# AIM-Harvard/pyradiomics

Measured on NVIDIA H100. Metric: voxels/s full-texture voxel-based, higher is better.
Workload: dtype f64

## Files before the change

### pyradiomics_b200/csrc/glrlm_fast.cuh

```cuda
#pragma once
#include "glcm_fast.cuh"

namespace rb {

struct GlrlmFastTables {
  uint32_t VA[GF_NA], VA2[GF_NA];
  uint8_t delta[GF_NA];
  double log2t[32];
  double clog2[32];
  double inv2[256];
};

inline void glrlm_fast_build_tables(GlrlmFastTables& T) {
  int ang[13][3], k = 0;
  for (int z = 1; z >= -1; z--) for (int y = 1; y >= -1; y--) for (int x = 1; x >= -1; x--)
    if (k < 13) { ang[k][0] = z; ang[k][1] = y; ang[k][2] = x; k++; }
  for (int a = 0; a < 13; a++) {
    T.VA[a] = T.VA2[a] = 0;
    T.delta[a] = (uint8_t)(ang[a][0] * 9 + ang[a][1] * 3 + ang[a][2]);
    for (int z = 0; z < 3; z++) for (int y = 0; y < 3; y++) for (int x = 0; x < 3; x++) {
      const int v = z * 9 + y * 3 + x;
      auto pos = [&](int m) {
        const int z2 = z + m * ang[a][0], y2 = y + m * ang[a][1], x2 = x + m * ang[a][2];
        return (z2 < 0 || z2 > 2 || y2 < 0 || y2 > 2 || x2 < 0 || x2 > 2) ? 31 : z2 * 9 + y2 * 3 + x2;
      };
      const int nx = pos(1), nx2 = pos(2);
      if (nx != 31) T.VA[a] |= 1u << v;
      if (nx2 != 31) T.VA2[a] |= 1u << v;
    }
  }
  T.log2t[0] = 0;
  T.clog2[0] = 0;
  for (int c = 1; c < 32; c++) { T.log2t[c] = log2((double)c); T.clog2[c] = c * log2((double)c); }
  T.inv2[0] = 0;
  for (int g = 1; g < 256; g++) T.inv2[g] = 1.0 / ((double)g * g);
}

RB_HD void glrlm_fast_voxel(const int* wl, const GlrlmFastTables& T, double* out) {
  uint32_t e[27];
  RB_EQMASKS_27(wl, e);
  uint32_t M = 0;
  uint32_t cls[13];
  int clg[13];
  int nl = 0;
  int S_n = 0, S_g = 0, S_g2 = 0;
  double S_ig = 0;
#pragma unroll
  for (int v = 0; v < 27; v++) {
    if (wl[v]) M |= 1u << v;
    if (e[v] && (e[v] & ((1u << v) - 1)) == 0) {
      if (e[v] == (1u << v)) { S_n++; S_g += wl[v]; S_g2 += wl[v] * wl[v]; S_ig += T.inv2[wl[v]]; }
      else { cls[nl] = e[v]; clg[nl] = wl[v]; nl++; }
    }
  }
  const int Np = RB_POPC(M);
  double sum[GLRLM_NF];
#pragma unroll
  for (int k = 0; k < GLRLM_NF; k++) sum[k] = 0;
  int nang = 0;
  for (int a = 0; a < GF_NA; a++) {
    const int d = T.delta[a];
    const uint32_t VA = T.VA[a];
    if (!(((M & VA) & (M >> d)) | ((M & T.VA2[a]) & (M >> (2 * d))))) continue;
    uint32_t NS = 0;
    for (int k = 0; k < nl; k++) NS |= cls[k] & (cls[k] >> d);
    NS &= VA;
    const uint32_t ENDS = M & ~NS, PS = NS << d, PS2 = PS & (PS << d);
    const uint32_t L1 = ENDS & ~PS, L2 = ENDS & PS & ~PS2, L3 = ENDS & PS2;
    const int n1 = RB_POPC(L1), n2 = RB_POPC(L2), n3 = RB_POPC(L3);
    int B1 = S_g2, B2 = 0, B3 = 0, C = S_g, sg = S_n;
    double A1 = S_ig, A2 = 0, A3 = 0, lg = 0;
    for (int k = 0; k < nl; k++) {
      const uint32_t E = cls[k];
      const int c1 = RB_POPC(E & L1), c2 = RB_POPC(E & L2), c3 = RB_POPC(E & L3), ce = c1 + c2 + c3;
      const int g = clg[k], g2 = g * g;
      const double ig = T.inv2[g];
      sg += ce * ce; C += ce * g;
      B1 += c1 * g2; B2 += c2 * g2; B3 += c3 * g2;
      A1 += c1 * ig; A2 += c2 * ig; A3 += c3 * ig;
      lg += T.clog2[c1] + T.clog2[c2] + T.clog2[c3];
    }
    const int Nr = n1 + n2 + n3;
    const double invNr = 1.0 / Nr, invNr2 = invNr * invNr;
    const int lre_n = n1 + 4 * n2 + 9 * n3, B = B1 + B2 + B3;
    sum[R_ShortRunEmphasis] += (n1 + n2 * 0.25 + n3 * (1.0 / 9.0)) * invNr;
    sum[R_LongRunEmphasis] += lre_n * invNr;
    sum[R_GrayLevelNonUniformity] += sg * invNr;
    sum[R_GrayLevelNonUniformityNormalized] += sg * invNr2;
    const int rl = n1 * n1 + n2 * n2 + n3 * n3;
    sum[R_RunLengthNonUniformity] += rl * invNr;
    sum[R_RunLengthNonUniformityNormalized] += rl * invNr2;
    sum[R_RunPercentage] += (double)Nr / Np;
    sum[R_GrayLevelVariance] += (double)(Nr * B - C * C) * invNr2;
    sum[R_RunVariance] += (double)(Nr * lre_n - Np * Np) * invNr2;
    sum[R_RunEntropy] += T.log2t[Nr] - lg * invNr;
    sum[R_LowGrayLevelRunEmphasis] += (A1 + A2 + A3) * invNr;
    sum[R_HighGrayLevelRunEmphasis] += B * invNr;
    sum[R_ShortRunLowGrayLevelEmphasis] += (A1 + A2 * 0.25 + A3 * (1.0 / 9.0)) * invNr;
    sum[R_ShortRunHighGrayLevelEmphasis] += (B1 + B2 * 0.25 + B3 * (1.0 / 9.0)) * invNr;
    sum[R_LongRunLowGrayLevelEmphasis] += (A1 + 4.0 * A2 + 9.0 * A3) * invNr;
    sum[R_LongRunHighGrayLevelEmphasis] += (double)(B1 + 4 * B2 + 9 * B3) * invNr;
    nang++;
  }
  const double inv = nang ? 1.0 / nang : NAN;
#pragma unroll
  for (int k = 0; k < GLRLM_NF; k++) out[k] = nang ? sum[k] * inv : NAN;
}

}
```

### pyradiomics_b200/csrc/small_fast.cuh

```cuda
#pragma once
#include "glcm_fast.cuh"

namespace rb {

struct SmallFastTables {
  double log2t[32];
  double inv2[256];
  double invsq[32];
  double rcp[64];
};

inline void small_fast_build_tables(SmallFastTables& T) {
  T.log2t[0] = 0; T.invsq[0] = 0; T.inv2[0] = 0; T.rcp[0] = 0;
  for (int c = 1; c < 32; c++) { T.log2t[c] = log2((double)c); T.invsq[c] = 1.0 / ((double)c * c); }
  for (int g = 1; g < 256; g++) T.inv2[g] = 1.0 / ((double)g * g);
  for (int c = 1; c < 64; c++) T.rcp[c] = 1.0 / (double)c;
}

RB_HD constexpr uint32_t nb26(int v) {
  uint32_t m = 0;
  const int z = v / 9, y = (v / 3) % 3, x = v % 3;
  for (int dz = -1; dz <= 1; dz++) for (int dy = -1; dy <= 1; dy++) for (int dx = -1; dx <= 1; dx++) {
    if (!dz && !dy && !dx) continue;
    const int z2 = z + dz, y2 = y + dy, x2 = x + dx;
    if (z2 < 0 || z2 > 2 || y2 < 0 || y2 > 2 || x2 < 0 || x2 > 2) continue;
    m |= 1u << (z2 * 9 + y2 * 3 + x2);
  }
  return m;
}
template <int V> struct NB26 { static constexpr uint32_t value = nb26(V); };

template <int V, int END> struct ForPos {
  template <typename F> static RB_HD void go(F& f) { f.template at<V>(); ForPos<V + 1, END>::go(f); }
};
template <int END> struct ForPos<END, END> { template <typename F> static RB_HD void go(F&) {} };

struct GldmPass1 {
  const int* wl; const uint32_t* cl; int* dep; uint32_t M;
  template <int V> RB_HD void at() { dep[V] = wl[V] ? (int)RB_POPC(cl[V] & NB26<V>::value) : -1 - V; }
};

RB_HD void gldm_fast_voxel(const int* wl, int alpha, const SmallFastTables& T, double* out) {
  uint32_t eq[27];
  RB_EQMASKS_27(wl, eq);
  uint32_t cl[27];
  if (alpha == 0) {
#pragma unroll
    for (int v = 0; v < 27; v++) cl[v] = eq[v];
  } else {
#pragma unroll
    for (int v = 0; v < 27; v++) cl[v] = 0;
#pragma unroll
    for (int p = 0; p < 27; p++)
#pragma unroll
      for (int q = p + 1; q < 27; q++) {
        const int d = wl[p] - wl[q];
        if (wl[p] && wl[q] && d <= alpha && -d <= alpha) { cl[p] |= 1u << q; cl[q] |= 1u << p; }
      }
  }
  int dep[27];
  GldmPass1 p1{wl, cl, dep, 0};
  ForPos<0, 27>::go(p1);
  uint32_t dq[27];
  RB_EQMASKS_27_KEY(dep, dq);
  int Nz = 0, Sj = 0, Sj2 = 0, B = 0, C = 0, X4 = 0, gl = 0, dn = 0;
  double Sinv = 0, A = 0, X1 = 0, X2 = 0, X3 = 0, lg = 0;
#pragma unroll
  for (int v = 0; v < 27; v++) {
    if (wl[v]) {
      const int g = wl[v], g2 = g * g, j = dep[v] + 1, j2 = j * j;
      const double ig = T.inv2[g], ij = T.invsq[j];
      Nz++; Sj += j; Sj2 += j2; B += g2; C += g; X4 += g2 * j2;
      Sinv += ij; A += ig; X1 += ig * ij; X2 += g2 * ij; X3 += j2 * ig;
      gl += RB_POPC(eq[v]); dn += RB_POPC(dq[v]);
      lg += T.log2t[RB_POPC(eq[v] & dq[v])];
    }
  }
  const double inv = 1.0 / Nz, inv2 = inv * inv;
  out[0] = T.log2t[Nz] - lg * inv;
  out[1] = dn * inv;
  out[2] = dn * inv2;
  out[3] = (double)(Nz * Sj2 - Sj * Sj) * inv2;
  out[4] = gl * inv;
  out[5] = (double)(Nz * B - C * C) * inv2;
  out[6] = B * inv;
  out[7] = Sj2 * inv;
  out[8] = X4 * inv;
  out[9] = X3 * inv;
  out[10] = A * inv;
  out[11] = Sinv * inv;
  out[12] = X2 * inv;
  out[13] = X1 * inv;
}

constexpr int NGTDM_L = 34034;

RB_HD constexpr int ngtdm_full_cnt(int v) {
  return (v % 3 == 1 ? 3 : 2) * ((v / 3) % 3 == 1 ? 3 : 2) * (v / 9 == 1 ? 3 : 2) - 1;
}

RB_HD double ngtdm_i2d(int d) {
#ifdef __CUDA_ARCH__
  return __hiloint2double(0x43300000, d) - 4503599627370496.0;
#else
  return (double)d;
#endif
}

RB_HD double ngtdm_complexity_pairs(const int* pk, const double* ns, int st, int nl, const SmallFastTables& T) {
  double c0 = 0, c1 = 0;
  for (int a = 0; a + 1 < nl; a++) {
    const int pa = pk[a * st], na = pa >> 8, ia = pa & 255;
    const double sa = ns[a * st];
    int b = a + 1;
    for (; b + 1 < nl; b += 2) {
      const int p0 = pk[b * st], p1 = pk[(b + 1) * st];
      const int x0 = ia - (p0 & 255), x1 = ia - (p1 & 255);
      c0 += ngtdm_i2d(x0 < 0 ? -x0 : x0) * ((sa + ns[b * st]) * T.rcp[na + (p0 >> 8)]);
      c1 += ngtdm_i2d(x1 < 0 ? -x1 : x1) * ((sa + ns[(b + 1) * st]) * T.rcp[na + (p1 >> 8)]);
    }
    if (b < nl) {
      const int p0 = pk[b * st], x0 = ia - (p0 & 255);
      c0 += ngtdm_i2d(x0 < 0 ? -x0 : x0) * ((sa + ns[b * st]) * T.rcp[na + (p0 >> 8)]);
    }
  }
  return c0 + c1;
}

struct NgtdmGeneralDiff {
  const int* wl; const uint32_t* eq; uint32_t M; const SmallFastTables* T; double* scr_ns; int st; double ssum;
  template <int V> RB_HD void at() {
    if (!wl[V]) return;
    constexpr uint32_t nb = NB26<V>::value;
    int sum = 0;
#pragma unroll
    for (int u = 0; u < 27; u++) if (nb >> u & 1u) sum += wl[u];
    const int cnt = RB_POPC(M & nb), x = cnt * wl[V] - sum;
    const double d = ngtdm_i2d(x < 0 ? -x : x) * T->rcp[cnt];
    ssum += d;
    const int r = RB_CTZ(eq[V]);
    const double prev = r == V ? 0.0 : scr_ns[r * st];
    scr_ns[r * st] = prev + d;
  }
};

template <bool FULL>
RB_HD void ngtdm_fast_body(const int* wl, const SmallFastTables& T, double* out, int* scr_pk, double* scr_ns, int st) {
  int B = 0, C = 0;
#pragma unroll
  for (int v = 0; v < 27; v++) { B += wl[v] * wl[v]; C += wl[v]; }
  uint32_t eq[27];
  RB_EQMASKS_27(wl, eq);
  int Nvp = 27, SE = 0;
  double ssum = 0;
  if (FULL) {
    int bx[27], by[27], bz[27];
#pragma unroll
    for (int r = 0; r < 27; r += 3) {
      bx[r] = wl[r] + wl[r + 1]; bx[r + 1] = bx[r] + wl[r + 2]; bx[r + 2] = wl[r + 1] + wl[r + 2];
    }
#pragma unroll
    for (int r = 0; r < 27; r += 9)
#pragma unroll
      for (int x = 0; x < 3; x++) {
        const int* b = bx + r + x;
        by[r + x] = b[0] + b[3]; by[r + 3 + x] = by[r + x] + b[6]; by[r + 6 + x] = b[3] + b[6];
      }
#pragma unroll
    for (int yx = 0; yx < 9; yx++) {
      bz[yx] = by[yx] + by[9 + yx]; bz[9 + yx] = bz[yx] + by[18 + yx]; bz[18 + yx] = by[9 + yx] + by[18 + yx];
    }
#pragma unroll
    for (int v = 0; v < 27; v++) {
      const int cnt = ngtdm_full_cnt(v);
      const int x = (cnt + 1) * wl[v] - bz[v];
      const int e = (x < 0 ? -x : x) * (NGTDM_L / cnt);
      SE += e;
      const int r = RB_CTZ(eq[v]);
      const int prev = r == v ? 0 : scr_pk[r * st];
      scr_pk[r * st] = prev + e;
    }
  } else {
    uint32_t M = 0;
#pragma unroll
    for (int v = 0; v < 27; v++) if (wl[v]) M |= 1u << v;
    Nvp = RB_POPC(M);
    NgtdmGeneralDiff p1{wl, eq, M, &T, scr_ns, st, 0.0};
    ForPos<0, 27>::go(p1);
    ssum = p1.ssum;
  }
  int nl = 0, SL = 0, SL2 = 0;
  double pw = 0;
  int X[27];
#pragma unroll
  for (int v = 0; v < 27; v++) {
    const bool rep = eq[v] && (eq[v] & ((1u << v) - 1)) == 0;
    const int n = RB_POPC(eq[v]), g = wl[v];
    const double ns = FULL ? ngtdm_i2d(n) * ngtdm_i2d(scr_pk[v * st]) : ngtdm_i2d(n) * scr_ns[v * st];
    scr_pk[nl * st] = n << 8 | g;
    scr_ns[nl * st] = ns;
    X[v] = rep ? g * n : 0;
    if (rep) { nl++; SL += g; SL2 += g * g; pw += ns; }
  }
  RB_NGTDM_SORT27(X);
  int bd = 0;
#pragma unroll
  for (int k = 0; k < 27; k++) bd += (2 * k - 53 + nl) * X[k];
  const double cpx = ngtdm_complexity_pairs(scr_pk, scr_ns, st, nl, T);
  const double u = FULL ? (double)NGTDM_L : 1.0, N = (double)Nvp;
  const double sdiff = FULL ? (double)SE : ssum;
  out[N_Coarseness] = pw != 0 ? N * u / pw : 1e6;
  const double div = (double)nl * (nl - 1);
  out[N_Contrast] = div != 0 ? 2.0 * (double)(Nvp * B - C * C) * sdiff / (N * N * N * u * div) : 0.0;
  out[N_Busyness] = bd != 0 ? pw / (2.0 * u * (double)bd) : 0.0;
  out[N_Complexity] = 2.0 * cpx / (N * u);
  out[N_Strength] = sdiff != 0 ? 2.0 * u * (double)(nl * B - 2 * C * SL + Nvp * SL2) / (N * sdiff) : 0.0;
}

RB_HD bool ngtdm_window_full(const int* wl) {
  bool full = true;
#pragma unroll
  for (int v = 0; v < 27; v++) full &= wl[v] != 0;
  return full;
}

RB_HD void ngtdm_fast_voxel(const int* wl, const SmallFastTables& T, double* out) {
  int pk[27] = {0};
  double ns[27] = {0};
  if (ngtdm_window_full(wl)) ngtdm_fast_body<true>(wl, T, out, pk, ns, 1);
  else ngtdm_fast_body<false>(wl, T, out, pk, ns, 1);
}

RB_HD uint32_t dilate26(uint32_t m) {
  constexpr uint32_t X0 = 0x1249249u, X2 = 0x4924924u;
  constexpr uint32_t Y0 = 0x01C0E07u, Y2 = 0x70381C0u;
  m |= ((m & ~X2) << 1) | ((m & ~X0) >> 1);
  m |= ((m & ~Y2) << 3) | ((m & ~Y0) >> 3);
  m |= (m << 9) | (m >> 9);
  return m & 0x7FFFFFFu;
}

struct GlszmAcc {
  int Nz, Sg, Sg2, Ss2, X4, gln;
  double A, Sinv, X1, X2, X3, lg;
  unsigned long long h0, h1, h2;
};

RB_HD void glszm_fast_voxel(const int* wl, const SmallFastTables& T, double* out) {
  uint32_t eq[27];
  RB_EQMASKS_27(wl, eq);
  uint32_t M = 0;
  uint32_t cls[13];
  int clg[13];
  int nl = 0, S_n = 0, S_g = 0, S_g2 = 0;
  double S_ig = 0;
#pragma unroll
  for (int v = 0; v < 27; v++) {
    if (wl[v]) M |= 1u << v;
    if (eq[v] && (eq[v] & ((1u << v) - 1)) == 0) {
      if (eq[v] == (1u << v)) { S_n++; S_g += wl[v]; S_g2 += wl[v] * wl[v]; S_ig += T.inv2[wl[v]]; }
      else { cls[nl] = eq[v]; clg[nl] = wl[v]; nl++; }
    }
  }
  GlszmAcc a;
  a.Nz = S_n; a.Sg = S_g; a.Sg2 = S_g2; a.Ss2 = S_n; a.X4 = S_g2; a.gln = S_n;
  a.A = S_ig; a.Sinv = (double)S_n; a.X1 = S_ig; a.X2 = (double)S_g2; a.X3 = S_ig; a.lg = 0;
  a.h0 = (unsigned long long)S_n; a.h1 = a.h2 = 0;
  for (int k = 0; k < nl; k++) {
    const int g = clg[k], g2 = g * g;
    uint32_t m = cls[k];
    const double ig = T.inv2[g];
    int zs[8];
    int zc = 0;
    while (m && zc < 8) {
      uint32_t comp = m & (0u - m);
      for (;;) {
        const uint32_t nx = dilate26(comp) & m;
        if (nx == comp) break;
        comp = nx;
      }
      m &= ~comp;
      const int sz = RB_POPC(comp), s2 = sz * sz;
      zs[zc++] = sz;
      const double is = T.invsq[sz];
      a.Nz++; a.Sg += g; a.Sg2 += g2; a.Ss2 += s2; a.X4 += g2 * s2;
      a.A += ig; a.Sinv += is; a.X1 += ig * is; a.X2 += g2 * is; a.X3 += s2 * ig;
      if (sz <= 12) a.h0 += 1ull << (5 * (sz - 1));
      else if (sz <= 24) a.h1 += 1ull << (5 * (sz - 13));
      else a.h2 += 1ull << (5 * (sz - 25));
    }
    a.gln += zc * zc;
    for (int k = 0; k < zc; k++) {
      int c = 0;
      for (int l = 0; l < zc; l++) c += zs[l] == zs[k];
      a.lg += T.log2t[c];
    }
  }
  int szn = 0;
#pragma unroll
  for (int k = 0; k < 12; k++) {
    const int c0 = (int)(a.h0 >> (5 * k)) & 31, c1 = (int)(a.h1 >> (5 * k)) & 31;
    szn += c0 * c0 + c1 * c1;
  }
#pragma unroll
  for (int k = 0; k < 3; k++) { const int c2 = (int)(a.h2 >> (5 * k)) & 31; szn += c2 * c2; }
  const int Np = RB_POPC(M), Nz = a.Nz;
  const double inv = 1.0 / Nz, inv2 = inv * inv;
  out[S_GLN] = a.gln * inv; out[S_GLNN] = a.gln * inv2;
  out[S_GLV] = (double)(Nz * a.Sg2 - a.Sg * a.Sg) * inv2;
  out[S_HGLE] = a.Sg2 * inv; out[S_LargeE] = a.Ss2 * inv; out[S_LargeHGLE] = a.X4 * inv; out[S_LargeLGLE] = a.X3 * inv;
  out[S_LGLE] = a.A * inv; out[S_SizeNU] = szn * inv; out[S_SizeNUN] = szn * inv2; out[S_SmallE] = a.Sinv * inv;
  out[S_SmallHGLE] = a.X2 * inv; out[S_SmallLGLE] = a.X1 * inv;
  out[S_Entropy] = T.log2t[Nz] - a.lg * inv;
  out[S_Percentage] = (double)Nz / Np;
  out[S_SizeVar] = (double)(Nz * a.Ss2 - Np * Np) * inv2;
}

}
```

### pyradiomics_b200/csrc/voxel_fast.cu

```cuda
#include <map>
#include <mutex>

#include "common.cuh"
#define RB_GLCM_BLOCK_SYNC 1
#include "glcm_fast.cuh"
#include "glcm_kernels.cuh"
#include "glrlm_fast.cuh"
#include "small_fast.cuh"
#include "host_common.hpp"

namespace rb {

bool glcm_fast_applicable(int cls, int level_bytes, const VoxParams& P) {
  return cls == C_GLCM && level_bytes == 1 && P.rz == 1 && P.ry == 1 && P.rx == 1 && P.na == 13 && P.symmetric &&
         !P.weighted && P.Ng <= 255;
}

struct GlcmQueue { GlcmTask* q = nullptr; double* res = nullptr; unsigned* count = nullptr; size_t cap = 0; };
static std::mutex g_queue_mu;
static std::map<std::pair<int, cudaStream_t>, GlcmQueue> g_queue_cache;
int glcm_release_queues() {
  int dev = 0;
  if (cudaGetDevice(&dev) != cudaSuccess) return RB_ERR_CUDA;
  cudaDeviceSynchronize();
  std::lock_guard<std::mutex> lk(g_queue_mu);
  for (auto it = g_queue_cache.begin(); it != g_queue_cache.end();) {
    if (it->first.first == dev) {
      cudaFree(it->second.q); cudaFree(it->second.res); cudaFree(it->second.count);
      it = g_queue_cache.erase(it);
    } else ++it;
  }
  return RB_OK;
}
static GlcmQueue* glcm_queue(cudaStream_t st, size_t need) {
  std::mutex& mu = g_queue_mu;
  auto& cache = g_queue_cache;
  int dev = 0;
  if (cudaGetDevice(&dev) != cudaSuccess) return nullptr;
  std::lock_guard<std::mutex> lk(mu);
  GlcmQueue& Q = cache[{dev, st}];
  if (!Q.count && cudaMalloc(&Q.count, sizeof(unsigned)) != cudaSuccess) return nullptr;
  if (Q.cap < need) {
    if (Q.q) { cudaStreamSynchronize(st); cudaFree(Q.q); cudaFree(Q.res); Q.q = nullptr; Q.res = nullptr; Q.cap = 0; }
    if (cudaMalloc(&Q.q, need * sizeof(GlcmTask)) != cudaSuccess) return nullptr;
    if (cudaMalloc(&Q.res, need * sizeof(double)) != cudaSuccess) { cudaFree(Q.q); Q.q = nullptr; return nullptr; }
    Q.cap = need;
  }
  return &Q;
}

int glcm_fast_launch(const void* lev, const uint8_t* centers, const VoxParams& P, double* out, long long fstride,
                     int z0, int z1, int out_z0, cudaStream_t st) {
  const GlcmFastTables* T = device_table<GlcmFastTables>([&](GlcmFastTables& h) { glcm_fast_build_tables(h, P.Ng); }, P.Ng);
  if (!T) return fail(RB_ERR_CUDA, "could not build the GLCM table block on the device");
  const long long plane = (long long)P.Y * P.X;
  if ((long long)(z1 - z0) * plane <= 0) return RB_OK;
  if (P.sy != P.X || P.sz != plane) return fail(RB_ERR_ARG, "GLCM fast path expects a contiguous level volume");
  const int sms = sm_count();
  const long long max_entries = 48ll << 20;
  int zchunk = (int)(max_entries / (plane * GF_NA));
  if (zchunk < 1) zchunk = 1;
  if (zchunk > z1 - z0) zchunk = z1 - z0;
  GlcmQueue* Q = glcm_queue(st, (size_t)zchunk * plane * GF_NA);
  if (!Q) return fail(RB_ERR_NOMEM, "could not allocate the GLCM eigen-task queue");
  constexpr int NT = 512;
  const int smem = glcm_phaseA_smem_bytes(NT);
  RB_CUDA(set_max_dynamic_smem(glcm_fast_kernel<1, NT>, smem));
  RB_CUDA(set_max_dynamic_smem(glcm_fast_solve_kernel<2>, GF_LZ_SMEM_BYTES));
  const uint8_t* l8 = (const uint8_t*)lev;
  for (int za = z0; za < z1; za += zchunk) {
    const int zb = za + zchunk < z1 ? za + zchunk : z1;
    RB_CUDA(cudaMemsetAsync(Q->count, 0, sizeof(unsigned), st));
    int grid = 0;
    RB_CUDA(resident_grid(glcm_fast_kernel<1, NT>, NT, smem, (long long)(zb - za) * plane, grid));
    glcm_fast_kernel<1, NT><<<grid, NT, smem, st>>>(l8, centers, P, T, out, fstride, za, zb, out_z0, Q->q, Q->count);
    RB_LAUNCH_CHECK();
    glcm_fast_solve_kernel<0><<<sms * 8, 128, 0, st>>>(l8, P, T, Q->q, Q->count, Q->res, 0);
    for (int g = 10; g <= 12; g += 2) glcm_fast_solve_kernel<1><<<sms * 8, 128, 0, st>>>(l8, P, T, Q->q, Q->count, Q->res, g);
    for (int g = 18; g >= 14; g -= 2)
      glcm_fast_solve_kernel<2><<<sms * 2, 128, GF_LZ_SMEM_BYTES, st>>>(l8, P, T, Q->q, Q->count, Q->res, g);
    RB_LAUNCH_CHECK();
    glcm_fast_finish_kernel<<<sms * 8, 256, 0, st>>>(P, Q->q, Q->count, Q->res, out + (long long)G_MCC * fstride, out_z0);
    RB_LAUNCH_CHECK();
  }
  return RB_OK;
}

__global__ void __launch_bounds__(128)
glrlm_fast_kernel(const uint8_t* __restrict__ lev, const uint8_t* __restrict__ centers,
                  const __grid_constant__ VoxParams P, const GlrlmFastTables* __restrict__ Tg,
                  double* __restrict__ out, long long fstride, int z0, int z1, int out_z0) {
  __shared__ GlrlmFastTables T;
  copy_tables_to_shared(T, Tg);
  __syncthreads();
  const long long plane = (long long)P.Y * P.X;
  const long long total = (long long)(z1 - z0) * plane;
  for (long long t = (long long)blockIdx.x * blockDim.x + threadIdx.x; t < total; t += (long long)gridDim.x * blockDim.x) {
    const ChunkVoxel v = chunk_voxel(P, plane, z0, out_z0, t);
    if (!chunk_center(lev, centers, plane, v)) {
#pragma unroll
      for (int k = 0; k < GLRLM_NF; k++) out[k * fstride + v.oi] = P.init_value;
      continue;
    }
    int wl[27];
    load_window27(lev, P, v.z, v.y, v.x, v.vi, true, wl, 1);
    double f[GLRLM_NF];
    glrlm_fast_voxel(wl, T, f);
#pragma unroll
    for (int k = 0; k < GLRLM_NF; k++) out[k * fstride + v.oi] = f[k];
  }
}

bool glrlm_fast_applicable(int cls, int level_bytes, const VoxParams& P) {
  return cls == C_GLRLM && level_bytes == 1 && P.rz == 1 && P.ry == 1 && P.rx == 1 && P.na == 13 && !P.weighted && P.Ng <= 255;
}

int glrlm_fast_launch(const void* lev, const uint8_t* centers, const VoxParams& P, double* out, long long fstride,
                      int z0, int z1, int out_z0, cudaStream_t st) {
  const GlrlmFastTables* T = device_table<GlrlmFastTables>(glrlm_fast_build_tables);
  if (!T) return fail(RB_ERR_CUDA, "could not build the GLRLM table block on the device");
  const long long total = (long long)(z1 - z0) * P.Y * P.X;
  if (total <= 0) return RB_OK;
  glrlm_fast_kernel<<<grid_for(total, 128, 32), 128, 0, st>>>((const uint8_t*)lev, centers, P, T, out, fstride, z0, z1, out_z0);
  RB_LAUNCH_CHECK();
  return RB_OK;
}

template <int CLS, int NT, bool SYNC>
__global__ void __launch_bounds__(NT)
small_fast_kernel(const uint8_t* __restrict__ lev, const uint8_t* __restrict__ centers,
                  const __grid_constant__ VoxParams P, const SmallFastTables* __restrict__ Tg,
                  double* __restrict__ out, long long fstride, int z0, int z1, int out_z0) {
  __shared__ SmallFastTables T;
  copy_tables_to_shared<NT>(T, Tg);
  __syncthreads();
  constexpr int NF = CLS == C_GLSZM ? GLSZM_NF : GLDM_NF;
  const long long plane = (long long)P.Y * P.X;
  const long long total = (long long)(z1 - z0) * plane;
  const long long ntiles = (total + NT - 1) / NT;
  for (long long tile = blockIdx.x; tile < ntiles; tile += gridDim.x) {
    if (SYNC) __syncthreads();
    const long long t = tile * NT + threadIdx.x;
    const bool live = t < total;
    if (!SYNC && !live) continue;
    const ChunkVoxel v = chunk_voxel(P, plane, z0, out_z0, t, live);
    const bool is_center = live && chunk_center(lev, centers, plane, v);
    if (!SYNC && !is_center) {
#pragma unroll
      for (int k = 0; k < NF; k++) out[k * fstride + v.oi] = P.init_value;
      continue;
    }
    int wl[27];
    load_window27(lev, P, v.z, v.y, v.x, v.vi, is_center, wl, 1);
    double f[16];
    if (CLS == C_GLSZM) glszm_fast_voxel(wl, T, f);
    else gldm_fast_voxel(wl, P.alpha, T, f);
    if (!live) continue;
#pragma unroll
    for (int k = 0; k < NF; k++) out[k * fstride + v.oi] = is_center ? f[k] : P.init_value;
  }
}

constexpr int NGTDM_NT = 128;
template <int NT>
__global__ void __launch_bounds__(NT, 4)
ngtdm_fast_kernel(const uint8_t* __restrict__ lev, const uint8_t* __restrict__ centers,
                  const __grid_constant__ VoxParams P, const SmallFastTables* __restrict__ Tg,
                  double* __restrict__ out, long long fstride, int z0, int z1, int out_z0) {
  __shared__ SmallFastTables T;
  __shared__ double ng_ns[27 * NT];
  __shared__ int ng_pk[27 * NT];
  __shared__ long long defer[2 * NT];
  __shared__ unsigned ndefer;
  copy_tables_to_shared<NT>(T, Tg);
  const int tid = threadIdx.x;
  if (tid == 0) ndefer = 0;
  __syncthreads();
  const long long plane = (long long)P.Y * P.X;
  full_window_tiles<NT>((long long)(z1 - z0) * plane, defer, ndefer,
    [&](long long t, bool live, auto defer_it) {
      if (!live) return;
      const ChunkVoxel v = chunk_voxel(P, plane, z0, out_z0, t);
      const bool is_center = chunk_center(lev, centers, plane, v);
      int wl[27];
      load_window27(lev, P, v.z, v.y, v.x, v.vi, is_center, wl, 1);
      if (is_center && ngtdm_window_full(wl)) {
        double f[NGTDM_NF];
        ngtdm_fast_body<true>(wl, T, f, ng_pk + tid, ng_ns + tid, NT);
#pragma unroll
        for (int k = 0; k < NGTDM_NF; k++) out[k * fstride + v.oi] = f[k];
      } else if (is_center) {
        defer_it();
      } else {
#pragma unroll
        for (int k = 0; k < NGTDM_NF; k++) out[k * fstride + v.oi] = P.init_value;
      }
    },
    [&](auto entry, bool live) {
      if (!live) return;
      const ChunkVoxel v = chunk_voxel(P, plane, z0, out_z0, entry());
      const bool is_center = chunk_center(lev, centers, plane, v);
      int wl[27];
      load_window27(lev, P, v.z, v.y, v.x, v.vi, is_center, wl, 1);
      double f[NGTDM_NF];
      ngtdm_fast_body<false>(wl, T, f, ng_pk + tid, ng_ns + tid, NT);
#pragma unroll
      for (int k = 0; k < NGTDM_NF; k++) out[k * fstride + v.oi] = f[k];
    });
}

bool small_fast_applicable(int cls, int level_bytes, const VoxParams& P) {
  return (cls == C_GLSZM || cls == C_GLDM || cls == C_NGTDM) && level_bytes == 1 && P.rz == 1 && P.ry == 1 && P.rx == 1 &&
         P.na == 26 && P.Ng <= 255;
}

int small_fast_launch(int cls, const void* lev, const uint8_t* centers, const VoxParams& P, double* out, long long fstride,
                      int z0, int z1, int out_z0, cudaStream_t st) {
  const SmallFastTables* T = device_table<SmallFastTables>(small_fast_build_tables);
  if (!T) return fail(RB_ERR_CUDA, "could not build the table block on the device");
  const long long total = (long long)(z1 - z0) * P.Y * P.X;
  if (total <= 0) return RB_OK;
  const uint8_t* l8 = (const uint8_t*)lev;
  if (cls == C_NGTDM) {
    int grid = 0;
    RB_CUDA(resident_grid(ngtdm_fast_kernel<NGTDM_NT>, NGTDM_NT, 0, total, grid));
    ngtdm_fast_kernel<NGTDM_NT><<<grid, NGTDM_NT, 0, st>>>(l8, centers, P, T, out, fstride, z0, z1, out_z0);
  } else if (cls == C_GLSZM) {
    small_fast_kernel<C_GLSZM, 128, false><<<grid_for(total, 128, 32), 128, 0, st>>>(l8, centers, P, T, out, fstride, z0, z1, out_z0);
  } else {
    small_fast_kernel<C_GLDM, 256, true><<<grid_for(total, 256, 16), 256, 0, st>>>(l8, centers, P, T, out, fstride, z0, z1, out_z0);
  }
  RB_LAUNCH_CHECK();
  return RB_OK;
}

}
```

Before: 263.9 million.

## Specialize GLRLM/GLSZM for full windows with deferred partial windows and shared scratch

Templates the GLRLM and GLSZM per-voxel bodies on a FULL flag so fully-populated 3x3x3 windows skip mask building and angle-skip tests. Both now run in the deferred-tile kernel used for NGTDM: partial-window voxels are queued and processed separately, which keeps warps convergent. Per-thread class masks move to strided shared memory to relieve registers. Reciprocal tables replace divisions, and GLSZM entropy uses an incremental nibble histogram instead of an O(n^2) recount. In exchange it adds shared-memory use and deferral synchronization, and the load_window27 return value is now treated as a fullness flag.

```diff
diff --git a/pyradiomics_b200/csrc/glrlm_fast.cuh b/pyradiomics_b200/csrc/glrlm_fast.cuh
--- a/pyradiomics_b200/csrc/glrlm_fast.cuh
+++ b/pyradiomics_b200/csrc/glrlm_fast.cuh
@@ -8,72 +8,76 @@
   uint8_t delta[GF_NA];
   double log2t[32];
   double clog2[32];
+  double rcp[32];
   double inv2[256];
 };
 
+RB_HD constexpr uint32_t glrlm_succ(int a, int m) {
+  const int dz = 1 - a / 9, dy = 1 - a / 3 % 3, dx = 1 - a % 3;
+  uint32_t r = 0;
+  for (int v = 0; v < 27; v++) {
+    const int z = v / 9 + m * dz, y = v / 3 % 3 + m * dy, x = v % 3 + m * dx;
+    if (z >= 0 && z <= 2 && y >= 0 && y <= 2 && x >= 0 && x <= 2) r |= 1u << v;
+  }
+  return r;
+}
+
 inline void glrlm_fast_build_tables(GlrlmFastTables& T) {
-  int ang[13][3], k = 0;
-  for (int z = 1; z >= -1; z--) for (int y = 1; y >= -1; y--) for (int x = 1; x >= -1; x--)
-    if (k < 13) { ang[k][0] = z; ang[k][1] = y; ang[k][2] = x; k++; }
-  for (int a = 0; a < 13; a++) {
-    T.VA[a] = T.VA2[a] = 0;
-    T.delta[a] = (uint8_t)(ang[a][0] * 9 + ang[a][1] * 3 + ang[a][2]);
-    for (int z = 0; z < 3; z++) for (int y = 0; y < 3; y++) for (int x = 0; x < 3; x++) {
-      const int v = z * 9 + y * 3 + x;
-      auto pos = [&](int m) {
-        const int z2 = z + m * ang[a][0], y2 = y + m * ang[a][1], x2 = x + m * ang[a][2];
-        return (z2 < 0 || z2 > 2 || y2 < 0 || y2 > 2 || x2 < 0 || x2 > 2) ? 31 : z2 * 9 + y2 * 3 + x2;
-      };
-      const int nx = pos(1), nx2 = pos(2);
-      if (nx != 31) T.VA[a] |= 1u << v;
-      if (nx2 != 31) T.VA2[a] |= 1u << v;
-    }
+  for (int a = 0; a < GF_NA; a++) {
+    T.VA[a] = glrlm_succ(a, 1); T.VA2[a] = glrlm_succ(a, 2); T.delta[a] = (uint8_t)(13 - a);
   }
   T.log2t[0] = 0;
   T.clog2[0] = 0;
-  for (int c = 1; c < 32; c++) { T.log2t[c] = log2((double)c); T.clog2[c] = c * log2((double)c); }
+  T.rcp[0] = 0;
+  for (int c = 1; c < 32; c++) {
+    T.log2t[c] = log2((double)c); T.clog2[c] = c * log2((double)c); T.rcp[c] = 1.0 / (double)c;
+  }
   T.inv2[0] = 0;
   for (int g = 1; g < 256; g++) T.inv2[g] = 1.0 / ((double)g * g);
 }
 
-RB_HD void glrlm_fast_voxel(const int* wl, const GlrlmFastTables& T, double* out) {
+template <bool FULL>
+RB_HD void glrlm_fast_body(const int* wl, const GlrlmFastTables& T, double* out, uint32_t* scr_cls, uint8_t* scr_g,
+                           int st) {
   uint32_t e[27];
   RB_EQMASKS_27(wl, e);
-  uint32_t M = 0;
-  uint32_t cls[13];
-  int clg[13];
+  uint32_t M = FULL ? 0x7FFFFFFu : 0u;
   int nl = 0;
   int S_n = 0, S_g = 0, S_g2 = 0;
   double S_ig = 0;
 #pragma unroll
   for (int v = 0; v < 27; v++) {
-    if (wl[v]) M |= 1u << v;
-    if (e[v] && (e[v] & ((1u << v) - 1)) == 0) {
+    if (!FULL && wl[v]) M |= 1u << v;
+    if ((FULL || e[v]) && (e[v] & ((1u << v) - 1)) == 0) {
       if (e[v] == (1u << v)) { S_n++; S_g += wl[v]; S_g2 += wl[v] * wl[v]; S_ig += T.inv2[wl[v]]; }
-      else { cls[nl] = e[v]; clg[nl] = wl[v]; nl++; }
+      else { scr_cls[nl * st] = e[v]; scr_g[nl * st] = (uint8_t)wl[v]; nl++; }
     }
   }
-  const int Np = RB_POPC(M);
+  const int Np = FULL ? 27 : RB_POPC(M);
   double sum[GLRLM_NF];
 #pragma unroll
   for (int k = 0; k < GLRLM_NF; k++) sum[k] = 0;
-  int nang = 0;
+  int nang = 0, SNr = 0;
+#pragma unroll 1
   for (int a = 0; a < GF_NA; a++) {
     const int d = T.delta[a];
     const uint32_t VA = T.VA[a];
-    if (!(((M & VA) & (M >> d)) | ((M & T.VA2[a]) & (M >> (2 * d))))) continue;
-    uint32_t NS = 0;
-    for (int k = 0; k < nl; k++) NS |= cls[k] & (cls[k] >> d);
-    NS &= VA;
-    const uint32_t ENDS = M & ~NS, PS = NS << d, PS2 = PS & (PS << d);
+    if (!FULL && !(((M & VA) & (M >> d)) | ((M & T.VA2[a]) & (M >> (2 * d))))) continue;
+    uint32_t NSa = 0;
+    for (int k = 0; k < nl; k++) {
+      const uint32_t E = scr_cls[k * st];
+      NSa |= E & (E >> d);
+    }
+    NSa &= VA;
+    const uint32_t ENDS = M & ~NSa, PS = NSa << d, PS2 = PS & (PS << d);
     const uint32_t L1 = ENDS & ~PS, L2 = ENDS & PS & ~PS2, L3 = ENDS & PS2;
     const int n1 = RB_POPC(L1), n2 = RB_POPC(L2), n3 = RB_POPC(L3);
     int B1 = S_g2, B2 = 0, B3 = 0, C = S_g, sg = S_n;
     double A1 = S_ig, A2 = 0, A3 = 0, lg = 0;
     for (int k = 0; k < nl; k++) {
-      const uint32_t E = cls[k];
+      const uint32_t E = scr_cls[k * st];
       const int c1 = RB_POPC(E & L1), c2 = RB_POPC(E & L2), c3 = RB_POPC(E & L3), ce = c1 + c2 + c3;
-      const int g = clg[k], g2 = g * g;
+      const int g = scr_g[k * st], g2 = g * g;
       const double ig = T.inv2[g];
       sg += ce * ce; C += ce * g;
       B1 += c1 * g2; B2 += c2 * g2; B3 += c3 * g2;
@@ -81,7 +85,7 @@
       lg += T.clog2[c1] + T.clog2[c2] + T.clog2[c3];
     }
     const int Nr = n1 + n2 + n3;
-    const double invNr = 1.0 / Nr, invNr2 = invNr * invNr;
+    const double invNr = T.rcp[Nr], invNr2 = invNr * invNr;
     const int lre_n = n1 + 4 * n2 + 9 * n3, B = B1 + B2 + B3;
     sum[R_ShortRunEmphasis] += (n1 + n2 * 0.25 + n3 * (1.0 / 9.0)) * invNr;
     sum[R_LongRunEmphasis] += lre_n * invNr;
@@ -90,7 +94,7 @@
     const int rl = n1 * n1 + n2 * n2 + n3 * n3;
     sum[R_RunLengthNonUniformity] += rl * invNr;
     sum[R_RunLengthNonUniformityNormalized] += rl * invNr2;
-    sum[R_RunPercentage] += (double)Nr / Np;
+    SNr += Nr;
     sum[R_GrayLevelVariance] += (double)(Nr * B - C * C) * invNr2;
     sum[R_RunVariance] += (double)(Nr * lre_n - Np * Np) * invNr2;
     sum[R_RunEntropy] += T.log2t[Nr] - lg * invNr;
@@ -102,9 +106,29 @@
     sum[R_LongRunHighGrayLevelEmphasis] += (double)(B1 + 4 * B2 + 9 * B3) * invNr;
     nang++;
   }
-  const double inv = nang ? 1.0 / nang : NAN;
+  if (!FULL && !nang) {
 #pragma unroll
-  for (int k = 0; k < GLRLM_NF; k++) out[k] = nang ? sum[k] * inv : NAN;
+    for (int k = 0; k < GLRLM_NF; k++) out[k] = NAN;
+    return;
+  }
+  sum[R_RunPercentage] = (double)SNr / (FULL ? 13.0 * 27.0 : (double)(nang * Np));
+  const double inv = FULL ? 1.0 / 13.0 : T.rcp[nang];
+#pragma unroll
+  for (int k = 0; k < GLRLM_NF; k++) out[k] = k == R_RunPercentage ? sum[k] : sum[k] * inv;
+}
+
+RB_HD bool glrlm_window_full(const int* wl) {
+  bool full = true;
+#pragma unroll
+  for (int v = 0; v < 27; v++) full &= wl[v] != 0;
+  return full;
+}
+
+RB_HD void glrlm_fast_voxel(const int* wl, const GlrlmFastTables& T, double* out) {
+  uint32_t cls[13];
+  uint8_t g[13];
+  if (glrlm_window_full(wl)) glrlm_fast_body<true>(wl, T, out, cls, g, 1);
+  else glrlm_fast_body<false>(wl, T, out, cls, g, 1);
 }
 
 }
diff --git a/pyradiomics_b200/csrc/small_fast.cuh b/pyradiomics_b200/csrc/small_fast.cuh
--- a/pyradiomics_b200/csrc/small_fast.cuh
+++ b/pyradiomics_b200/csrc/small_fast.cuh
@@ -8,6 +8,7 @@
   double inv2[256];
   double invsq[32];
   double rcp[64];
+  double zlg[8];
 };
 
 inline void small_fast_build_tables(SmallFastTables& T) {
@@ -15,6 +16,7 @@
   for (int c = 1; c < 32; c++) { T.log2t[c] = log2((double)c); T.invsq[c] = 1.0 / ((double)c * c); }
   for (int g = 1; g < 256; g++) T.inv2[g] = 1.0 / ((double)g * g);
   for (int c = 1; c < 64; c++) T.rcp[c] = 1.0 / (double)c;
+  for (int c = 0; c < 8; c++) T.zlg[c] = (c + 1) * T.log2t[c + 1] - c * T.log2t[c];
 }
 
 RB_HD constexpr uint32_t nb26(int v) {
@@ -217,7 +219,7 @@
   out[N_Strength] = sdiff != 0 ? 2.0 * u * (double)(nl * B - 2 * C * SL + Nvp * SL2) / (N * sdiff) : 0.0;
 }
 
-RB_HD bool ngtdm_window_full(const int* wl) {
+RB_HD bool window27_full(const int* wl) {
   bool full = true;
 #pragma unroll
   for (int v = 0; v < 27; v++) full &= wl[v] != 0;
@@ -227,7 +229,7 @@
 RB_HD void ngtdm_fast_voxel(const int* wl, const SmallFastTables& T, double* out) {
   int pk[27] = {0};
   double ns[27] = {0};
-  if (ngtdm_window_full(wl)) ngtdm_fast_body<true>(wl, T, out, pk, ns, 1);
+  if (window27_full(wl)) ngtdm_fast_body<true>(wl, T, out, pk, ns, 1);
   else ngtdm_fast_body<false>(wl, T, out, pk, ns, 1);
 }
 
@@ -246,20 +248,20 @@
   unsigned long long h0, h1, h2;
 };
 
-RB_HD void glszm_fast_voxel(const int* wl, const SmallFastTables& T, double* out) {
+template <bool FULL>
+RB_HD void glszm_fast_body(const int* wl, const SmallFastTables& T, double* out, uint32_t* scr_cls, uint8_t* scr_g,
+                           int st) {
   uint32_t eq[27];
   RB_EQMASKS_27(wl, eq);
-  uint32_t M = 0;
-  uint32_t cls[13];
-  int clg[13];
+  uint32_t M = FULL ? 0x7FFFFFFu : 0u;
   int nl = 0, S_n = 0, S_g = 0, S_g2 = 0;
   double S_ig = 0;
 #pragma unroll
   for (int v = 0; v < 27; v++) {
-    if (wl[v]) M |= 1u << v;
-    if (eq[v] && (eq[v] & ((1u << v) - 1)) == 0) {
+    if (!FULL && wl[v]) M |= 1u << v;
+    if ((FULL || eq[v]) && (eq[v] & ((1u << v) - 1)) == 0) {
       if (eq[v] == (1u << v)) { S_n++; S_g += wl[v]; S_g2 += wl[v] * wl[v]; S_ig += T.inv2[wl[v]]; }
-      else { cls[nl] = eq[v]; clg[nl] = wl[v]; nl++; }
+      else { scr_cls[nl * st] = eq[v]; scr_g[nl * st] = (uint8_t)wl[v]; nl++; }
     }
   }
   GlszmAcc a;
@@ -267,12 +269,12 @@
   a.A = S_ig; a.Sinv = (double)S_n; a.X1 = S_ig; a.X2 = (double)S_g2; a.X3 = S_ig; a.lg = 0;
   a.h0 = (unsigned long long)S_n; a.h1 = a.h2 = 0;
   for (int k = 0; k < nl; k++) {
-    const int g = clg[k], g2 = g * g;
-    uint32_t m = cls[k];
+    const int g = scr_g[k * st], g2 = g * g;
+    uint32_t m = scr_cls[k * st];
     const double ig = T.inv2[g];
-    int zs[8];
+    unsigned long long lh = 0;
     int zc = 0;
-    while (m && zc < 8) {
+    while (m) {
       uint32_t comp = m & (0u - m);
       for (;;) {
         const uint32_t nx = dilate26(comp) & m;
@@ -281,20 +283,20 @@
       }
       m &= ~comp;
       const int sz = RB_POPC(comp), s2 = sz * sz;
-      zs[zc++] = sz;
+      zc++;
       const double is = T.invsq[sz];
       a.Nz++; a.Sg += g; a.Sg2 += g2; a.Ss2 += s2; a.X4 += g2 * s2;
       a.A += ig; a.Sinv += is; a.X1 += ig * is; a.X2 += g2 * is; a.X3 += s2 * ig;
       if (sz <= 12) a.h0 += 1ull << (5 * (sz - 1));
       else if (sz <= 24) a.h1 += 1ull << (5 * (sz - 13));
       else a.h2 += 1ull << (5 * (sz - 25));
+      if (sz <= 13) {
+        const int sh = 4 * (sz - 1);
+        a.lg += T.zlg[(int)(lh >> sh) & 15];
+        lh += 1ull << sh;
+      }
     }
     a.gln += zc * zc;
-    for (int k = 0; k < zc; k++) {
-      int c = 0;
-      for (int l = 0; l < zc; l++) c += zs[l] == zs[k];
-      a.lg += T.log2t[c];
-    }
   }
   int szn = 0;
 #pragma unroll
@@ -304,16 +306,23 @@
   }
 #pragma unroll
   for (int k = 0; k < 3; k++) { const int c2 = (int)(a.h2 >> (5 * k)) & 31; szn += c2 * c2; }
-  const int Np = RB_POPC(M), Nz = a.Nz;
-  const double inv = 1.0 / Nz, inv2 = inv * inv;
+  const int Np = FULL ? 27 : RB_POPC(M), Nz = a.Nz;
+  const double inv = T.rcp[Nz], inv2 = inv * inv;
   out[S_GLN] = a.gln * inv; out[S_GLNN] = a.gln * inv2;
   out[S_GLV] = (double)(Nz * a.Sg2 - a.Sg * a.Sg) * inv2;
   out[S_HGLE] = a.Sg2 * inv; out[S_LargeE] = a.Ss2 * inv; out[S_LargeHGLE] = a.X4 * inv; out[S_LargeLGLE] = a.X3 * inv;
   out[S_LGLE] = a.A * inv; out[S_SizeNU] = szn * inv; out[S_SizeNUN] = szn * inv2; out[S_SmallE] = a.Sinv * inv;
   out[S_SmallHGLE] = a.X2 * inv; out[S_SmallLGLE] = a.X1 * inv;
   out[S_Entropy] = T.log2t[Nz] - a.lg * inv;
-  out[S_Percentage] = (double)Nz / Np;
+  out[S_Percentage] = Nz * T.rcp[Np];
   out[S_SizeVar] = (double)(Nz * a.Ss2 - Np * Np) * inv2;
 }
 
-}
+RB_HD void glszm_fast_voxel(const int* wl, const SmallFastTables& T, double* out) {
+  uint32_t cls[13];
+  uint8_t g[13];
+  if (window27_full(wl)) glszm_fast_body<true>(wl, T, out, cls, g, 1);
+  else glszm_fast_body<false>(wl, T, out, cls, g, 1);
+}
+
+}
diff --git a/pyradiomics_b200/csrc/voxel_fast.cu b/pyradiomics_b200/csrc/voxel_fast.cu
--- a/pyradiomics_b200/csrc/voxel_fast.cu
+++ b/pyradiomics_b200/csrc/voxel_fast.cu
@@ -1,5 +1,6 @@
 #include <map>
 #include <mutex>
+#include <type_traits>
 
 #include "common.cuh"
 #define RB_GLCM_BLOCK_SYNC 1
@@ -86,29 +87,58 @@
   return RB_OK;
 }
 
-__global__ void __launch_bounds__(128)
-glrlm_fast_kernel(const uint8_t* __restrict__ lev, const uint8_t* __restrict__ centers,
-                  const __grid_constant__ VoxParams P, const GlrlmFastTables* __restrict__ Tg,
-                  double* __restrict__ out, long long fstride, int z0, int z1, int out_z0) {
-  __shared__ GlrlmFastTables T;
-  copy_tables_to_shared(T, Tg);
+constexpr int RLSZ_NT = 128;
+template <int CLS> using RlszTables = std::conditional_t<CLS == C_GLRLM, GlrlmFastTables, SmallFastTables>;
+
+template <int CLS, int NT>
+__global__ void __launch_bounds__(NT, 4)
+glrlm_glszm_fast_kernel(const uint8_t* __restrict__ lev, const uint8_t* __restrict__ centers,
+                        const __grid_constant__ VoxParams P, const RlszTables<CLS>* __restrict__ Tg,
+                        double* __restrict__ out, long long fstride, int z0, int z1, int out_z0) {
+  constexpr int NF = CLS == C_GLRLM ? GLRLM_NF : GLSZM_NF;
+  __shared__ RlszTables<CLS> T;
+  __shared__ uint32_t cl_mask[13 * NT];
+  __shared__ uint8_t cl_level[13 * NT];
+  __shared__ long long defer[2 * NT];
+  __shared__ unsigned ndefer;
+  copy_tables_to_shared<NT>(T, Tg);
+  const int tid = threadIdx.x;
+  if (tid == 0) ndefer = 0;
   __syncthreads();
   const long long plane = (long long)P.Y * P.X;
-  const long long total = (long long)(z1 - z0) * plane;
-  for (long long t = (long long)blockIdx.x * blockDim.x + threadIdx.x; t < total; t += (long long)gridDim.x * blockDim.x) {
-    const ChunkVoxel v = chunk_voxel(P, plane, z0, out_z0, t);
-    if (!chunk_center(lev, centers, plane, v)) {
-#pragma unroll
-      for (int k = 0; k < GLRLM_NF; k++) out[k * fstride + v.oi] = P.init_value;
-      continue;
-    }
-    int wl[27];
-    load_window27(lev, P, v.z, v.y, v.x, v.vi, true, wl, 1);
-    double f[GLRLM_NF];
-    glrlm_fast_voxel(wl, T, f);
-#pragma unroll
-    for (int k = 0; k < GLRLM_NF; k++) out[k * fstride + v.oi] = f[k];
-  }
+  auto body = [&](auto full, const int* wl, double* f) {
+    if constexpr (CLS == C_GLRLM) glrlm_fast_body<decltype(full)::value>(wl, T, f, cl_mask + tid, cl_level + tid, NT);
+    else glszm_fast_body<decltype(full)::value>(wl, T, f, cl_mask + tid, cl_level + tid, NT);
+  };
+  full_window_tiles<NT>((long long)(z1 - z0) * plane, defer, ndefer,
+    [&](long long t, bool live, auto defer_it) {
+      if (!live) return;
+      const ChunkVoxel v = chunk_voxel(P, plane, z0, out_z0, t);
+      const bool is_center = chunk_center(lev, centers, plane, v);
+      int wl[27];
+      const bool full = load_window27(lev, P, v.z, v.y, v.x, v.vi, is_center, wl, 1);
+      if (full) {
+        double f[NF];
+        body(std::true_type(), wl, f);
+#pragma unroll
+        for (int k = 0; k < NF; k++) out[k * fstride + v.oi] = f[k];
+      } else if (is_center) {
+        defer_it();
+      } else {
+#pragma unroll
+        for (int k = 0; k < NF; k++) out[k * fstride + v.oi] = P.init_value;
+      }
+    },
+    [&](auto entry, bool live) {
+      if (!live) return;
+      const ChunkVoxel v = chunk_voxel(P, plane, z0, out_z0, entry());
+      int wl[27];
+      load_window27(lev, P, v.z, v.y, v.x, v.vi, true, wl, 1);
+      double f[NF];
+      body(std::false_type(), wl, f);
+#pragma unroll
+      for (int k = 0; k < NF; k++) out[k * fstride + v.oi] = f[k];
+    });
 }
 
 bool glrlm_fast_applicable(int cls, int level_bytes, const VoxParams& P) {
@@ -121,43 +151,38 @@
   if (!T) return fail(RB_ERR_CUDA, "could not build the GLRLM table block on the device");
   const long long total = (long long)(z1 - z0) * P.Y * P.X;
   if (total <= 0) return RB_OK;
-  glrlm_fast_kernel<<<grid_for(total, 128, 32), 128, 0, st>>>((const uint8_t*)lev, centers, P, T, out, fstride, z0, z1, out_z0);
+  int grid = 0;
+  RB_CUDA(resident_grid(glrlm_glszm_fast_kernel<C_GLRLM, RLSZ_NT>, RLSZ_NT, 0, total, grid));
+  glrlm_glszm_fast_kernel<C_GLRLM, RLSZ_NT><<<grid, RLSZ_NT, 0, st>>>((const uint8_t*)lev, centers, P, T, out, fstride, z0,
+                                                                   z1, out_z0);
   RB_LAUNCH_CHECK();
   return RB_OK;
 }
 
-template <int CLS, int NT, bool SYNC>
+template <int NT>
 __global__ void __launch_bounds__(NT)
-small_fast_kernel(const uint8_t* __restrict__ lev, const uint8_t* __restrict__ centers,
-                  const __grid_constant__ VoxParams P, const SmallFastTables* __restrict__ Tg,
-                  double* __restrict__ out, long long fstride, int z0, int z1, int out_z0) {
+gldm_fast_kernel(const uint8_t* __restrict__ lev, const uint8_t* __restrict__ centers,
+                 const __grid_constant__ VoxParams P, const SmallFastTables* __restrict__ Tg,
+                 double* __restrict__ out, long long fstride, int z0, int z1, int out_z0) {
   __shared__ SmallFastTables T;
   copy_tables_to_shared<NT>(T, Tg);
   __syncthreads();
-  constexpr int NF = CLS == C_GLSZM ? GLSZM_NF : GLDM_NF;
   const long long plane = (long long)P.Y * P.X;
   const long long total = (long long)(z1 - z0) * plane;
   const long long ntiles = (total + NT - 1) / NT;
   for (long long tile = blockIdx.x; tile < ntiles; tile += gridDim.x) {
-    if (SYNC) __syncthreads();
+    __syncthreads();
     const long long t = tile * NT + threadIdx.x;
     const bool live = t < total;
-    if (!SYNC && !live) continue;
     const ChunkVoxel v = chunk_voxel(P, plane, z0, out_z0, t, live);
     const bool is_center = live && chunk_center(lev, centers, plane, v);
-    if (!SYNC && !is_center) {
-#pragma unroll
-      for (int k = 0; k < NF; k++) out[k * fstride + v.oi] = P.init_value;
-      continue;
-    }
     int wl[27];
     load_window27(lev, P, v.z, v.y, v.x, v.vi, is_center, wl, 1);
-    double f[16];
-    if (CLS == C_GLSZM) glszm_fast_voxel(wl, T, f);
-    else gldm_fast_voxel(wl, P.alpha, T, f);
+    double f[GLDM_NF];
+    gldm_fast_voxel(wl, P.alpha, T, f);
     if (!live) continue;
 #pragma unroll
-    for (int k = 0; k < NF; k++) out[k * fstride + v.oi] = is_center ? f[k] : P.init_value;
+    for (int k = 0; k < GLDM_NF; k++) out[k * fstride + v.oi] = is_center ? f[k] : P.init_value;
   }
 }
 
@@ -184,7 +209,7 @@
       const bool is_center = chunk_center(lev, centers, plane, v);
       int wl[27];
       load_window27(lev, P, v.z, v.y, v.x, v.vi, is_center, wl, 1);
-      if (is_center && ngtdm_window_full(wl)) {
+      if (is_center && window27_full(wl)) {
         double f[NGTDM_NF];
         ngtdm_fast_body<true>(wl, T, f, ng_pk + tid, ng_ns + tid, NT);
 #pragma unroll
@@ -226,9 +251,11 @@
     RB_CUDA(resident_grid(ngtdm_fast_kernel<NGTDM_NT>, NGTDM_NT, 0, total, grid));
     ngtdm_fast_kernel<NGTDM_NT><<<grid, NGTDM_NT, 0, st>>>(l8, centers, P, T, out, fstride, z0, z1, out_z0);
   } else if (cls == C_GLSZM) {
-    small_fast_kernel<C_GLSZM, 128, false><<<grid_for(total, 128, 32), 128, 0, st>>>(l8, centers, P, T, out, fstride, z0, z1, out_z0);
+    int grid = 0;
+    RB_CUDA(resident_grid(glrlm_glszm_fast_kernel<C_GLSZM, RLSZ_NT>, RLSZ_NT, 0, total, grid));
+    glrlm_glszm_fast_kernel<C_GLSZM, RLSZ_NT><<<grid, RLSZ_NT, 0, st>>>(l8, centers, P, T, out, fstride, z0, z1, out_z0);
   } else {
-    small_fast_kernel<C_GLDM, 256, true><<<grid_for(total, 256, 16), 256, 0, st>>>(l8, centers, P, T, out, fstride, z0, z1, out_z0);
+    gldm_fast_kernel<256><<<grid_for(total, 256, 16), 256, 0, st>>>(l8, centers, P, T, out, fstride, z0, z1, out_z0);
   }
   RB_LAUNCH_CHECK();
   return RB_OK;
```

After: 266.2 million, median of 6. No clear change (+0.9%).
